# xinpw8/pokegym

Hardware: NVIDIA B200
Metric: env_steps_per_s (higher is better)
Workload: dtype u8

## Files before the change

pokegym_b200/csrc/gb_classes.inc:

```
#if defined(GB_CLS)
GB_CLS(0, 4, 0x2000u)
GB_CLS(1, 6, 0x1000u)
GB_CLS(2, 11, 0x0000u)
GB_CLS(3, 2, 0x4020u)
GB_CLS(4, 0, 0x0800u)
GB_CLS(5, 0, 0x0a00u)
GB_CLS(6, 3, 0x0000u)
GB_CLS(7, 0, 0x08a0u)
GB_CLS(8, 1, 0x0020u)
GB_CLS(9, 2, 0x4010u)
GB_CLS(10, 0, 0x0810u)
GB_CLS(11, 1, 0x0000u)
GB_CLS(12, 3, 0x0010u)
GB_CLS(13, 0, 0x0a80u)
GB_CLS(14, 0, 0x0820u)
GB_CLS(15, 9, 0x0000u)
GB_CLS(16, 10, 0x0160u)
GB_CLS(17, 1, 0x0200u)
GB_CLS(18, 8, 0x0160u)
GB_CLS(19, 7, 0x0000u)
GB_CLS(20, 3, 0x0020u)
GB_CLS(21, 4, 0x2220u)
GB_CLS(22, 8, 0x0560u)
GB_CLS(23, 12, 0x0000u)
GB_CLS(24, 2, 0x4000u)
GB_CLS(25, 14, 0x0000u)
GB_CLS(26, 5, 0x0000u)
GB_CLS(27, 15, 0x0000u)
GB_CLS(28, 13, 0x0000u)
GB_CLS(29, 16, 0x0000u)
GB_CLS(30, 0, 0x0a10u)
GB_CLS(31, 11, 0x0220u)
GB_CLS(32, 12, 0x0020u)
GB_CLS(33, 13, 0x0220u)
#endif
#define GB_CLS_COUNT 34
#define GB_CLS_DISPATCH(c, L, OTHER) \
if (GB_CLS_TEST((c) < 3u)) { \
    if (GB_CLS_TEST((c) == 0u)) { \
      L(0, 4, 0x2000u) \
    } else { \
        if (GB_CLS_TEST((c) == 1u)) { \
          L(1, 6, 0x1000u) \
        } else { \
              L(2, 11, 0x0000u) \
        } \
    } \
} else { \
    if (GB_CLS_TEST((c) < 6u)) { \
        if (GB_CLS_TEST((c) == 3u)) { \
          L(3, 2, 0x4020u) \
        } else { \
            if (GB_CLS_TEST((c) == 4u)) { \
              L(4, 0, 0x0800u) \
            } else { \
                  L(5, 0, 0x0a00u) \
            } \
        } \
    } else { \
        if (GB_CLS_TEST((c) < 8u)) { \
            if (GB_CLS_TEST((c) == 6u)) { \
              L(6, 3, 0x0000u) \
            } else { \
                  L(7, 0, 0x08a0u) \
            } \
        } else { \
            if (GB_CLS_TEST((c) < 11u)) { \
                if (GB_CLS_TEST((c) == 8u)) { \
                  L(8, 1, 0x0020u) \
                } else { \
                    if (GB_CLS_TEST((c) == 9u)) { \
                      L(9, 2, 0x4010u) \
                    } else { \
                          L(10, 0, 0x0810u) \
                    } \
                } \
            } else { \
                if (GB_CLS_TEST((c) < 14u)) { \
                    if (GB_CLS_TEST((c) == 11u)) { \
                      L(11, 1, 0x0000u) \
                    } else { \
                        if (GB_CLS_TEST((c) == 12u)) { \
                          L(12, 3, 0x0010u) \
                        } else { \
                              L(13, 0, 0x0a80u) \
                        } \
                    } \
                } else { \
                    if (GB_CLS_TEST((c) < 17u)) { \
                        if (GB_CLS_TEST((c) == 14u)) { \
                          L(14, 0, 0x0820u) \
                        } else { \
                            if (GB_CLS_TEST((c) == 15u)) { \
                              L(15, 9, 0x0000u) \
                            } else { \
                                  L(16, 10, 0x0160u) \
                            } \
                        } \
                    } else { \
                        if (GB_CLS_TEST((c) < 20u)) { \
                            if (GB_CLS_TEST((c) == 17u)) { \
                              L(17, 1, 0x0200u) \
                            } else { \
                                if (GB_CLS_TEST((c) == 18u)) { \
                                  L(18, 8, 0x0160u) \
                                } else { \
                                      L(19, 7, 0x0000u) \
                                } \
                            } \
                        } else { \
                            if (GB_CLS_TEST((c) < 22u)) { \
                                if (GB_CLS_TEST((c) == 20u)) { \
                                  L(20, 3, 0x0020u) \
                                } else { \
                                      L(21, 4, 0x2220u) \
                                } \
                            } else { \
                                if (GB_CLS_TEST((c) == 22u)) { \
                                  L(22, 8, 0x0560u) \
                                } else { \
                                    if (GB_CLS_TEST((c) == 23u)) { \
                                      L(23, 12, 0x0000u) \
                                    } else { \
                                        if (GB_CLS_TEST((c) == 24u)) { \
                                          L(24, 2, 0x4000u) \
                                        } else { \
                                            if (GB_CLS_TEST((c) == 25u)) { \
                                              L(25, 14, 0x0000u) \
                                            } else { \
                                                if (GB_CLS_TEST((c) == 26u)) { \
                                                  L(26, 5, 0x0000u) \
                                                } else { \
                                                    if (GB_CLS_TEST((c) == 27u)) { \
                                                      L(27, 15, 0x0000u) \
                                                    } else { \
                                                        if (GB_CLS_TEST((c) == 28u)) { \
                                                          L(28, 13, 0x0000u) \
                                                        } else { \
                                                            if (GB_CLS_TEST((c) == 29u)) { \
                                                              L(29, 16, 0x0000u) \
                                                            } else { \
                                                                if (GB_CLS_TEST((c) < 33u)) { \
                                                                    if (GB_CLS_TEST((c) == 30u)) { \
                                                                      L(30, 0, 0x0a10u) \
                                                                    } else { \
                                                                        if (GB_CLS_TEST((c) == 31u)) { \
                                                                          L(31, 11, 0x0220u) \
                                                                        } else { \
                                                                              L(32, 12, 0x0020u) \
                                                                        } \
                                                                    } \
                                                                } else { \
                                                                    if (GB_CLS_TEST((c) == 33u)) { \
                                                                      L(33, 13, 0x0220u) \
                                                                    } else { \
                                                                      OTHER \
                                                                    } \
                                                                } \
                                                            } \
                                                        } \
                                                    } \
                                                } \
                                            } \
                                        } \
                                    } \
                                } \
                            } \
                        } \
                    } \
                } \
            } \
        } \
    } \
} \
```

pokegym_b200/csrc/gb_cpu.cuh:

```cuda
#pragma once
#include "gb_device.cuh"
#include "gb_predecode.h"

#if !defined(GB_TRACE_SLOT)
#define GB_TRACE_SLOT(kind, phys, dx, dw)
#endif

__constant__ uint4 c_base_desc[512];

#define MODE_ATTN 0x8000u
#define MODE_POST 0x10000u
#define MODE_DEFER 0x20000u

struct RunCtx {
    const uint4 *rom_dec;
    uint32_t bank_mask;
};

__device__ __forceinline__ uint32_t hot_mode(const Machine &m) {
    const uint32_t attn = m.halted | m.iq | (m.iflag & m.ie & 0x1F), post = m.halted;
    return (attn ? MODE_ATTN : 0u) | (post ? MODE_POST : 0u) | (m.defer_active ? MODE_DEFER : 0u);
}
#define TIMA_ON 0x04000000u
__device__ __forceinline__ int hot_rem(Machine &m, bool fresh) {
    int rem = lcd_deadline(m);
    if (m.tmr & TIMA_ON) {
        int rt = (int)timer_divider(M_TAC(m)) - (int)m.timac;
        if (fresh) rt = rt < 1 ? 1 : rt;
        rem = rt < rem ? rt : rem;
    }
    return rem;
}
__device__ __forceinline__ void time_sync(Machine &m, int rem) {
    const uint32_t e = (uint32_t)(m.t_sync - rem);
    m.clock += e;
    m.divc += e;
    if (m.tmr & TIMA_ON) m.timac += e;
    m.t_sync = rem;
}

__global__ void k_predecode_rom(const uint8_t *rom, uint32_t rom_len, uint4 *out) {
    uint32_t o = blockIdx.x * blockDim.x + threadIdx.x;
    if (o >= rom_len) return;
    uint32_t in_bank = o & 0x3FFF;
    if (in_bank >= 0x3FFD) {
        out[o] = make_uint4(H_SLOW, 0, 0x32103210u, PD_NO_CLASS_W);
        return;
    }
    uint32_t ins = rom[o] | (rom[o + 1] << 8) | (rom[o + 2] << 16);
    out[o] = pd_finish(c_base_desc[(ins & 0xFF) == 0xCB ? (256u | ((ins >> 8) & 0xFF)) : (ins & 0xFF)], ins, o < 0x4000 ? o : 0x4000 + in_bank);
}

__device__ GB_NOINLINE uint4 cpu_decode_slow(Machine &m, uint32_t pc) {
    uint32_t ins = 0;
    if (pc - 0xFF80u < 0x7Du) {
        const uint32_t i = MEM_HI + (pc - 0xFE00), w0 = mem_rd_word(m, i >> 2), w1 = mem_rd_word(m, (i >> 2) + 1), sh = (i & 3) * 8;
        ins = sh ? ((w0 >> sh) | (w1 << (32 - sh))) : w0;
    } else {
        for (uint32_t i = 0; i < 3; i++) ins |= bus_read_full(m, (pc + i) & 0xFFFF) << (8 * i);
    }
    return pd_finish(c_base_desc[(ins & 0xFF) == 0xCB ? (256u | ((ins >> 8) & 0xFF)) : (ins & 0xFF)], ins, pc);
}

__device__ GB_NOINLINE uint32_t cpu_attention(Machine &m) {
    if (!m.iq) {
        const uint32_t pending = m.iflag & m.ie & 0x1F;
        if (pending) {
            const uint32_t bit = pending & (0u - pending);
            if (m.halted) m.pc = (m.pc + 1) & 0xFFFF;
            if (m.ime) {
                m.iflag ^= bit;
                bus_write_full(m, (m.sp - 1) & 0xFFFF, m.pc >> 8);
                bus_write_full(m, (m.sp - 2) & 0xFFFF, m.pc & 0xFF);
                m.sp = (m.sp - 2) & 0xFFFF;
                m.pc = 0x40 + 8 * (31 - __clz(bit));
                m.ime = 0;
            }
            m.iq = 1;
            m.halted = 0;
            return 0;
        }
    } else if (m.halted) {
        m.halted = 0;
        m.pc = (m.pc + 1) & 0xFFFF;
    }
    if (m.halted) return 4u << 8;
    m.iq = 0;
    return 1;
}

__device__ GB_NOINLINE uint32_t cpu_post_slow(Machine &m, uint32_t cycles) {
    if (m.halted) {
        const bool sleeps_on = (m.lcdc & 0x80) && !(m.iflag & m.ie & 0x1F);
        const int a = sleeps_on ? lcd_deadline(m) : (int)(m.target - m.clock), b = timer_cycles_to_interrupt(m), c = a < b ? a : b;
        cycles = c < 0 ? 0u : (uint32_t)c;
        if ((m.tmr & 0x04000000u) && b <= 0 && !(m.iflag & m.ie & 0x1F)) {
            const uint32_t n = 0xFFu - M_TIMA(m);
            m.timac -= n * timer_divider(M_TAC(m));
            m.tmr |= 0xFF00u;
        }
    }
    timer_tick_tima(m, cycles);
    return cycles;
}


struct CpuRegs {
    uint32_t bcde, hlaf, sp, pc;
};

#define FAST_WR_NONE 0xFFFFFFFFu
#define FAST_WR_DROP 0xFFFFFFFEu
#define FAST_WR_BANK 0xFFFFFFFDu
#define FAST_WR_P1 0xFFFFFFFCu
__device__ __forceinline__ uint32_t mem_offset(uint32_t i) { return ((i >> 2) << 7) | (i & 3); }
__device__ __forceinline__ uint32_t fast_store_target(uint32_t a) {
    if (a - 0xC000u < 0x3E00u) return mem_offset(MEM_WRAM + (a & 0x1FFF));
    if (a - 0xFF80u < 0x7Fu || a - 0xFE00u < 0x100u) return mem_offset(MEM_HI + (a - 0xFE00));
    if (a - 0x8000u < 0x2000u) return mem_offset(MEM_VRAM + (a - 0x8000));
    if (a - 0x2000u < 0x2000u) return FAST_WR_BANK;
    if (a - 0xFF10u < 0x30u) return FAST_WR_DROP;
    if (a == 0xFF00u) return FAST_WR_P1;
    return FAST_WR_NONE;
}
__device__ __forceinline__ bool fast_plain_offset(uint32_t a, uint32_t &off) {
    const bool wram = a - 0xC000u < 0x3E00u, vram = a - 0x8000u < 0x2000u;
    const bool hi = (a - 0xFE00u < 0x100u) | (a - 0xFF80u < 0x7Fu);
    const uint32_t i = wram ? MEM_WRAM + (a & 0x1FFF) : a + (vram ? MEM_VRAM - 0x8000u : MEM_HI - 0xFE00u);
    off = mem_offset(i);
    return wram | vram | hi;
}
__device__ __forceinline__ uint32_t fast_load_u8(const uint8_t *base, uint32_t off, bool ok, uint32_t otherwise) {
#if defined(GB_HOSTSIM)
    return ok ? base[off] : otherwise;
#else
    uint32_t r = otherwise;
    asm volatile("{\n\t.reg .pred p;\n\tsetp.ne.u32 p, %2, 0;\n\t@p ld.global.u8 %0, [%1];\n\t}" : "+r"(r) : "l"(base + off), "r"((uint32_t)ok) : "memory");
    return r;
#endif
}
__device__ __forceinline__ bool fast_stack_push(uint32_t sp) { return sp - 0xC002u < 0x3DFFu; }

template <bool FAST, bool SIMT, int CH = -1, uint32_t CF = 0>
__device__ __forceinline__ bool cpu_exec(Machine &m, const uint4 d, CpuRegs &r, uint32_t &rom_off, uint32_t &mode, uint32_t &cyc, uint8_t *memb,
                                         const uint8_t *rom, uint32_t bank_mask, bool declined = false) {
    uint32_t bcde = r.bcde, hlaf = r.hlaf, sp = r.sp;
#define FAST_DECLINE()         \
    do {                       \
        if (!SIMT) return false; \
        declined = true;       \
    } while (0)
    auto rd8 = [&](uint32_t a) -> uint32_t {
        if (FAST) {
            if (a - 0xC000u < 0x3E00u) return memb[mem_offset(MEM_WRAM + (a & 0x1FFF))];
            if (a < 0x8000u) return __ldg(rom + (a + (a >> 14) * rom_off));
            if (a - 0xFF80u < 0x7Fu || a - 0xFF00u < 4u) return memb[mem_offset(MEM_HI + (a - 0xFE00))];
            declined = true;
            return 0;
        }
        return bus_read_full(m, a);
    };
    const uint32_t w = d.w, wf = CH >= 0 ? CF : d.w, h = CH >= 0 ? (uint32_t)CH : (d.x & 0xFF);
    uint32_t v = gb_prmt(bcde, hlaf, w);
    if (wf & PDF_IMM) v = d.y & 0xFFFFu;
    uint32_t wa = 0, wt = 0;
    if (wf & (PDF_RD | PDF_WR)) {
        wa = (wf & PDF_AIMM) ? (d.y & 0xFFFFu) : (gb_prmt(bcde, hlaf, w >> 16) & 0xFFFFu);
        if (wf & PDF_ASP) wa = sp;
        if (FAST && SIMT) {
            uint32_t off;
            const bool plain = fast_plain_offset(wa, off);
            if (wf & PDF_WR) {
                wt = plain ? off : (wa - 0x2000u < 0x2000u) ? FAST_WR_BANK : (wa - 0xFF10u < 0x30u) ? FAST_WR_DROP : wa == 0xFF00u ? FAST_WR_P1 : FAST_WR_NONE;
                if (wt == FAST_WR_NONE) FAST_DECLINE();
                if ((mode & MODE_DEFER) && (wa - 0x8000u < 0x2000u || wa - 0xFE00u < 0x100u)) FAST_DECLINE();
            }
            if (wf & PDF_RD) {
                const bool in_rom = wa < 0x8000u, ok = plain | in_rom | (wa - 0xFF00u < 4u);
                v = fast_load_u8(in_rom ? rom : memb, in_rom ? wa + (wa >> 14) * rom_off : off, ok, v);
                if (!ok) declined = true;
                if (wf & PDF_RD16) {
                    const uint32_t wb = (wa + 1) & 0xFFFF;
                    uint32_t off2;
                    const bool plain2 = fast_plain_offset(wb, off2), in_rom2 = wb < 0x8000u, ok2 = plain2 | in_rom2 | (wb - 0xFF00u < 4u);
                    v |= fast_load_u8(in_rom2 ? rom : memb, in_rom2 ? wb + (wb >> 14) * rom_off : off2, ok2, 0) << 8;
                    if (!ok2) declined = true;
                }
            }
        } else {
            if (FAST && (wf & PDF_WR)) {
                wt = fast_store_target(wa);
                if (wt == FAST_WR_NONE) FAST_DECLINE();
                if ((mode & MODE_DEFER) && (wa - 0x8000u < 0x2000u || wa - 0xFE00u < 0x100u)) FAST_DECLINE();
            }
            if (wf & PDF_RD) {
                v = rd8(wa);
                if (wf & PDF_RD16) v |= rd8((wa + 1) & 0xFFFF) << 8;
                if (FAST && declined) return false;
            }
        }
    }
    const uint32_t imm16 = d.y & 0xFFFFu, op = gb_prmt(d.x, 0, 0x4441), ex = gb_prmt(d.x, 0, 0x4442), f = hlaf >> 24;
    uint32_t rv = v, next_pc = d.y >> 16, wv = v, wn = wf & PDF_WR;
    cyc = d.x >> 24;
#define PAIR_OPERAND() (gb_prmt(bcde, hlaf, w >> 16) & 0xFFFFu)
    const bool jump_taken = SIMT && (wf & PDF_JUMP) && ((f ^ ex) & op) == 0;
    if (SIMT) {
        next_pc = jump_taken ? imm16 : next_pc;
        cyc += jump_taken ? (ex & 0xF) : 0u;
    }
    if ((wf & PDF_MOV) || (SIMT && (wf & PDF_JUMP)) || (FAST && SIMT && declined)) {
    } else if (!SIMT && (wf & PDF_JUMP)) {
        if (((f ^ ex) & op) == 0) { next_pc = imm16; cyc += ex & 0xF; }
    } else if (!SIMT && (wf & PDF_INCDEC)) {
        const uint32_t b = v & 0xFF, sum = b + op, res = sum & 0xFF;
        const uint32_t nf = (f & FLAG_C) | ((((b ^ op ^ sum) & 0x10) << 1) ^ ex) | (res == 0 ? FLAG_Z : 0);
        rv = res | (nf << 8);
        wv = res;
    } else if (wf & (PDF_INCDEC | PDF_ARITH)) {
        const bool inc = SIMT && (wf & PDF_INCDEC) != 0;
        const uint32_t b = v & 0xFF;
        const uint32_t a = inc ? b : ((hlaf >> 16) & 0xFF), x = inc ? op : (b ^ ex);
        const uint32_t cin = inc ? 0u : ((((f >> 4) & op) ^ ex) & 1);
        const uint32_t sum = a + x + cin, res = sum & 0xFF;
        const uint32_t hn = (((a ^ x ^ sum) & 0x10) << 1) ^ (ex & 0x60);
        const uint32_t cb = inc ? (f & FLAG_C) : (((sum >> 4) ^ ex) & 0x10);
        rv = res | ((hn | cb | (res == 0 ? FLAG_Z : 0)) << 8);
        wv = res;
    } else if (h == H_HLI) {
        rv = ((PAIR_OPERAND() + gb_prmt(d.x, 0, 0x9991)) & 0xFFFFu) | (v << 16);
    } else switch (h) {
    case H_LOGIC: {
        const uint32_t a = (hlaf >> 16) & 0xFF, b = v & 0xFF;
        const uint32_t res = ((a & b) & ex) | ((a ^ b) & op);
        rv = res | (((op ? 0 : FLAG_H) | (res == 0 ? FLAG_Z : 0)) << 8);
        break;
    }
    case H_ADD_HL: {
        const uint32_t hl = hlaf & 0xFFFF, ar = PAIR_OPERAND(), t = hl + ar;
        const uint32_t nf = (f & FLAG_Z) | (((hl & 0xFFF) + (ar & 0xFFF)) > 0xFFF ? FLAG_H : 0) | (t > 0xFFFF ? FLAG_C : 0);
        rv = (t & 0xFFFF) | (nf << 24);
        break;
    }
    case H_CALL: {
        if (((f ^ ex) & op) == 0) {
            if (FAST && !fast_stack_push(sp)) FAST_DECLINE();
            wa = (sp - 1) & 0xFFFF;
            if (FAST) wt = mem_offset(MEM_WRAM + (wa & 0x1FFF));
            wv = gb_prmt(next_pc, 0, 0x4401);
            wn = 2;
            sp = (sp - 2) & 0xFFFF;
            next_pc = imm16;
            cyc += ex & 0xF;
        }
        break;
    }
    case H_RET: {
        if (wf & PDF_RETI) m.ime = 1;
        if (((f ^ ex) & op) == 0) {
            next_pc = v & 0xFFFF;
            sp = (sp + 2) & 0xFFFF;
            cyc += ex & 0xF;
        }
        break;
    }
    case H_PUSH:
        if (FAST && !fast_stack_push(sp)) FAST_DECLINE();
        wa = (sp - 1) & 0xFFFF;
        if (FAST) wt = mem_offset(MEM_WRAM + (wa & 0x1FFF));
        wv = gb_prmt(PAIR_OPERAND(), 0, 0x4401);
        wn = 2;
        sp = (sp - 2) & 0xFFFF;
        break;
    case H_POP:
        rv = v & (0xFF00u | op);
        sp = (sp + 2) & 0xFFFF;
        break;
    case H_ROT: {
        const uint32_t b = v & 0xFF, c = (f >> 4) & 1, right = ex & 1, b7 = b >> 7;
        uint32_t cout = right ? (b & 1) : b7;
        const uint32_t in = (((ex >> 1) & cout) | ((ex >> 2) & c) | ((ex >> 3) & b7)) & 1;
        uint32_t res = right ? ((b >> 1) | (in << 7)) : (((b << 1) | in) & 0xFF);
        if (ex & 0x10) { res = ((b >> 4) | (b << 4)) & 0xFF; cout = 0; }
        const uint32_t nf = ((res == 0 && !(op & 8)) ? FLAG_Z : 0) | (cout << 4);
        rv = res | (nf << 8);
        wv = res;
        break;
    }
    case H_CPL: rv = (~(hlaf >> 16) & 0xFF) | ((f | FLAG_N | FLAG_H) << 8); break;
    case H_IME: m.ime = op; break;
    case H_JPHL: next_pc = hlaf & 0xFFFF; break;
    case H_BIT: rv = ((f & FLAG_C) | FLAG_H | ((v & imm16 & 0xFF) ? 0 : FLAG_Z)) << 8; break;
    case H_RESSET:
        rv = (v & imm16 & 0xFF) | (imm16 >> 8);
        wv = rv;
        break;
    default: {
        if (FAST) {
            FAST_DECLINE();
            break;
        }
        const uint32_t a = (hlaf >> 16) & 0xFF, hl = hlaf & 0xFFFF;
        switch (op) {
        case 0x76: m.halted = 1; mode |= MODE_ATTN | MODE_POST; next_pc = r.pc; break;
        case 0x10: break;
        case 0xF3: m.ime = 0; break;
        case 0xFB: m.ime = 1; break;
        case 0x27: {
            uint32_t corr = ((f & FLAG_H) ? 0x06 : 0) | ((f & FLAG_C) ? 0x60 : 0), t = a;
            if (f & FLAG_N) {
                t -= corr;
            } else {
                if ((t & 0x0F) > 9) corr |= 0x06;
                if (t > 0x99) corr |= 0x60;
                t += corr;
            }
            t &= 0xFF;
            hlaf = (hlaf & 0xFFFF) | (t << 16) | (((f & FLAG_N) | (t == 0 ? FLAG_Z : 0) | ((corr & 0x60) ? FLAG_C : 0)) << 24);
            break;
        }
        case 0x2F: hlaf = (hlaf & 0xFFFF) | ((~a & 0xFF) << 16) | ((f | FLAG_N | FLAG_H) << 24); break;
        case 0x37: hlaf = (hlaf & 0x00FFFFFFu) | (((f & FLAG_Z) | FLAG_C) << 24); break;
        case 0x3F: hlaf = (hlaf & 0x00FFFFFFu) | (((f & FLAG_Z) | ((f & FLAG_C) ^ FLAG_C)) << 24); break;
        case 0x08: wa = imm16; wv = sp; wn = 3; break;
        case 0xE8:
        case 0xF8: {
            const uint32_t imm8 = imm16 & 0xFF;
            const uint32_t nf = (((sp & 0xF) + (imm8 & 0xF)) > 0xF ? FLAG_H : 0) | (((sp & 0xFF) + imm8) > 0xFF ? FLAG_C : 0);
            const uint32_t t = (sp + ((imm8 ^ 0x80) - 0x80)) & 0xFFFF;
            hlaf = (hlaf & 0x00FFFFFFu) | (nf << 24);
            if (op == 0xE8) sp = t;
            else hlaf = (hlaf & 0xFFFF0000u) | t;
            break;
        }
        case 0xE9: next_pc = hl; break;
        case 0xF9: sp = hl; break;
        case 0x31: sp = imm16; break;
        case 0x33: sp = (sp + 1) & 0xFFFF; break;
        case 0x3B: sp = (sp + 0xFFFF) & 0xFFFF; break;
        case 0x39: {
            const uint32_t t = hl + sp;
            const uint32_t nf = (f & FLAG_Z) | (((hl & 0xFFF) + (sp & 0xFFF)) > 0xFFF ? FLAG_H : 0) | (t > 0xFFFF ? FLAG_C : 0);
            hlaf = (hlaf & 0x00FF0000u) | (t & 0xFFFF) | (nf << 24);
            break;
        }
        case 0xE2: wa = 0xFF00u | (bcde & 0xFF); wv = a; wn = PDF_WR; break;
        case 0xF2: hlaf = (hlaf & 0xFF00FFFFu) | (bus_read_full(m, 0xFF00u | (bcde & 0xFF)) << 16); break;
        default: m.fault = 1; break;
        }
        break;
    }
    }
#undef PAIR_OPERAND
#if !defined(GB_HOSTSIM) && !defined(GB_OPT_NO_JOIN)
    if (FAST && SIMT) {
        uint32_t dj = declined;
        asm volatile("" : "+r"(dj));
        declined = dj != 0;
    }
#endif
    if (FAST && declined) return false;
#undef FAST_DECLINE
    r.bcde = gb_prmt(bcde, rv, d.z);
    r.hlaf = gb_prmt(hlaf, rv, d.z >> 16);
    r.sp = sp;
    r.pc = next_pc;
    if (wn) {
        if (FAST) {
            if (wt < FAST_WR_P1) {
                memb[wt] = (uint8_t)wv;
                if (wn == 2) memb[mem_offset(MEM_WRAM + ((wa - 1) & 0x1FFF))] = (uint8_t)(wv >> 8);
            } else if (wt == FAST_WR_P1) {
                memb[mem_offset(MEM_HI + 0x100)] = (uint8_t)joypad_pull(m, wv & 0xFF);
            } else if (wt == FAST_WR_BANK) {
                uint32_t bank = wv & 0x7F;
                bank = bank ? bank : 1;
                m.rombank = bank;
                rom_off = (bank_mask ? (bank & bank_mask) : (bank % m.rom_banks)) * 0x4000u - 0x4000u;
                m.rom_off = rom_off;
            }
        } else {
            const uint32_t count = (wn & 3) ? 2u : 1u, second = (wn == 2 ? wa - 1 : wa + 1) & 0xFFFF;
            for (uint32_t i = 0; i < count; i++) bus_write_full(m, i ? second : wa, (i ? wv >> 8 : wv) & 0xFF);
        }
    }
    return true;
}

__device__ __forceinline__ void gb_opaque(uint32_t &v) {
#if !defined(GB_HOSTSIM)
    asm volatile("" : "+r"(v));
#endif
}
__device__ __forceinline__ bool cpu_exec_by_class(Machine &m, const uint4 d, CpuRegs &r, uint32_t &rom_off, uint32_t &mode, uint32_t &cyc, uint8_t *memb,
                                                  const uint8_t *rom, uint32_t bank_mask) {
    uint32_t c = PD_CLASS(d.w);
#define GB_CLS_TEST(t) (gb_opaque(c), (t))
#define GB_CLS_RUN(id, H, F) return cpu_exec<true, false, H, F>(m, d, r, rom_off, mode, cyc, memb, rom, bank_mask);
    GB_CLS_DISPATCH(c, GB_CLS_RUN, return false;)
#undef GB_CLS_RUN
#undef GB_CLS_TEST
}

__device__ __forceinline__ bool cpu_exec_lockstep(Machine &m, const uint4 d, CpuRegs &r, uint32_t &rom_off, uint32_t mode, uint32_t &cyc, uint8_t *memb,
                                                  const uint8_t *rom, uint32_t bank_mask, bool declined) {
    const uint32_t bcde = r.bcde, hlaf = r.hlaf, sp = r.sp;
    const uint32_t w = d.w, h = d.x & 0xFF, op = gb_prmt(d.x, 0, 0x4441), ex = gb_prmt(d.x, 0, 0x4442), imm16 = d.y & 0xFFFFu, fall = d.y >> 16;
    const uint32_t f = hlaf >> 24, a8 = (hlaf >> 16) & 0xFF, hl = hlaf & 0xFFFF;
    declined |= h >= H_RARE;
    const bool cond = ((f ^ ex) & op) == 0;
    const bool is_call = h == H_CALL, is_ret = h == H_RET, is_push = h == H_PUSH, is_pop = h == H_POP;
    const bool jumps = cond && ((w & PDF_JUMP) || is_call), returns = cond && is_ret, pushes = (cond && is_call) || is_push;
    uint32_t v = gb_prmt(bcde, hlaf, w);
    v = (w & PDF_IMM) ? imm16 : v;
    const uint32_t pair = gb_prmt(bcde, hlaf, w >> 16) & 0xFFFFu;
    uint32_t wa = (w & PDF_AIMM) ? imm16 : pair;
    wa = (w & PDF_ASP) ? sp : wa;
    wa = pushes ? ((sp - 1) & 0xFFFF) : wa;
    uint32_t off;
    const bool plain = fast_plain_offset(wa, off);
    const bool rd = (w & PDF_RD) != 0, rd16 = (w & PDF_RD16) != 0, wr = (w & PDF_WR) != 0;
    const bool wr_special = wr && !plain;
    const uint32_t wt = (wa - 0x2000u < 0x2000u) ? FAST_WR_BANK : (wa - 0xFF10u < 0x30u) ? FAST_WR_DROP : wa == 0xFF00u ? FAST_WR_P1 : FAST_WR_NONE;
    declined |= wr_special && wt == FAST_WR_NONE;
    declined |= pushes && !fast_stack_push(sp);
    declined |= wr && (mode & MODE_DEFER) && (wa - 0x8000u < 0x2000u || wa - 0xFE00u < 0x100u);
    const bool in_rom = wa < 0x8000u, rd_ok = plain || in_rom || (wa - 0xFF00u < 4u), rd16_ok = sp - 0xC000u < 0x3DFFu;
    declined |= (rd && !rd_ok) || (rd16 && !rd16_ok);
    v = fast_load_u8(in_rom ? rom : memb, in_rom ? wa + (wa >> 14) * rom_off : off, rd && rd_ok, v);
    v |= fast_load_u8(memb, mem_offset(MEM_WRAM + ((sp + 1) & 0x1FFF)), rd16 && rd16_ok, 0) << 8;
    const uint32_t b = v & 0xFF, b7 = b >> 7;
    const bool inc = (w & PDF_INCDEC) != 0;
    const uint32_t ad_a = inc ? b : a8, ad_x = inc ? op : (b ^ ex), ad_c = inc ? 0u : ((((f >> 4) & op) ^ ex) & 1);
    const uint32_t sum = ad_a + ad_x + ad_c, ad_res = sum & 0xFF;
    const uint32_t ad_f = ((((ad_a ^ ad_x ^ sum) & 0x10) << 1) ^ (ex & 0x60)) | (inc ? (f & FLAG_C) : (((sum >> 4) ^ ex) & 0x10)) | (ad_res == 0 ? FLAG_Z : 0);
    const uint32_t lg_res = ((a8 & b) & ex) | ((a8 ^ b) & op);
    const uint32_t lg_f = (op ? 0 : FLAG_H) | (lg_res == 0 ? FLAG_Z : 0);
    const uint32_t right = ex & 1;
    uint32_t rt_c = right ? (b & 1) : b7;
    const uint32_t rt_in = (((ex >> 1) & rt_c) | ((ex >> 2) & (f >> 4)) | ((ex >> 3) & b7)) & 1;
    uint32_t rt_res = right ? ((b >> 1) | (rt_in << 7)) : (((b << 1) | rt_in) & 0xFF);
    rt_res = (ex & 0x10) ? (((b >> 4) | (b << 4)) & 0xFF) : rt_res;
    rt_c = (ex & 0x10) ? 0u : rt_c;
    const uint32_t rt_f = ((rt_res == 0 && !(op & 8)) ? FLAG_Z : 0) | (rt_c << 4);
    const uint32_t hli = ((pair + gb_prmt(d.x, 0, 0x9991)) & 0xFFFFu) | (v << 16);
    const uint32_t t16 = hl + pair;
    const uint32_t addhl = (t16 & 0xFFFF) | (((f & FLAG_Z) | (((hl & 0xFFF) + (pair & 0xFFF)) > 0xFFF ? FLAG_H : 0) | (t16 > 0xFFFF ? FLAG_C : 0)) << 24);
    uint32_t rv = v;
    rv = (w & (PDF_INCDEC | PDF_ARITH)) ? (ad_res | (ad_f << 8)) : rv;
    rv = h == H_LOGIC ? (lg_res | (lg_f << 8)) : rv;
    rv = h == H_ROT ? (rt_res | (rt_f << 8)) : rv;
    rv = h == H_BIT ? (((f & FLAG_C) | FLAG_H | ((b & imm16) ? 0 : FLAG_Z)) << 8) : rv;
    rv = h == H_RESSET ? ((b & imm16) | (imm16 >> 8)) : rv;
    rv = h == H_CPL ? ((~a8 & 0xFF) | ((f | FLAG_N | FLAG_H) << 8)) : rv;
    rv = h == H_HLI ? hli : rv;
    rv = h == H_ADD_HL ? addhl : rv;
    rv = is_pop ? (v & (0xFF00u | op)) : rv;
    uint32_t next_pc = jumps ? imm16 : fall;
    next_pc = returns ? (v & 0xFFFF) : next_pc;
    next_pc = h == H_JPHL ? hl : next_pc;
    cyc = (d.x >> 24) + ((jumps || returns) ? (ex & 0xF) : 0u);
    const uint32_t new_sp = (sp + ((is_pop || returns) ? 2u : 0u) - (pushes ? 2u : 0u)) & 0xFFFF;
    uint32_t wv = h == H_HLI ? v : rv;
    wv = pushes ? gb_prmt(is_push ? pair : fall, 0, 0x4401) : wv;
    if (declined) return false;
    r.bcde = gb_prmt(bcde, rv, d.z);
    r.hlaf = gb_prmt(hlaf, rv, d.z >> 16);
    r.sp = new_sp;
    r.pc = next_pc;
    if ((wr && plain) || pushes) memb[off] = (uint8_t)wv;
    if (pushes) memb[mem_offset(MEM_WRAM + ((sp - 2) & 0x1FFF))] = (uint8_t)(wv >> 8);
    if (wr_special) {
        if (wt == FAST_WR_P1) {
            memb[mem_offset(MEM_HI + 0x100)] = (uint8_t)joypad_pull(m, wv & 0xFF);
        } else if (wt == FAST_WR_BANK) {
            uint32_t bank = wv & 0x7F;
            bank = bank ? bank : 1;
            m.rombank = bank;
            rom_off = (bank_mask ? (bank & bank_mask) : (bank % m.rom_banks)) * 0x4000u - 0x4000u;
            m.rom_off = rom_off;
        }
    }
    if ((w & PDF_RETI) || h == H_IME) m.ime = h == H_IME ? op : 1u;
    return true;
}

__device__ GB_NOINLINE uint32_t cpu_tick_slow(Machine &m, const uint4 *__restrict__ rom_dec, uint32_t bank_mask, uint32_t &timer_ticked) {
    uint32_t cyc = 0;
    bool execute = true;
    if (m.halted | m.iq | (m.iflag & m.ie & 0x1F)) {
        const uint32_t r = cpu_attention(m);
        execute = r & 1;
        cyc = r >> 8;
    }
    if (execute) {
        const uint32_t pc = m.pc;
        uint4 d = make_uint4(H_SLOW, 0, 0, PD_NO_CLASS_W);
        if (pc < 0x8000u) d = __ldg(rom_dec + (pc + (pc >> 14) * m.rom_off));
        if ((d.x & 0xFF) == H_SLOW) d = cpu_decode_slow(m, pc);
        CpuRegs r = {m.bcde, m.hlaf, m.sp, pc};
        uint32_t rom_off = m.rom_off, mode = 0;
        cpu_exec<false, false>(m, d, r, rom_off, mode, cyc, m.memb, m.rom, bank_mask);
        m.bcde = r.bcde; m.hlaf = r.hlaf; m.sp = r.sp; m.pc = r.pc;
        m.n_instr++;
    }
    timer_ticked = m.halted;
    if (m.halted) cyc = cpu_post_slow(m, cyc);
    return cyc;
}

__device__ __forceinline__ uint4 cpu_decode_hram(const uint8_t *memb, uint32_t pc) {
    const uint32_t i = MEM_HI + (pc - 0xFE00), sh = (i & 3) * 8;
    const uint32_t w0 = ((const uint32_t *)memb)[(i >> 2) << 5], w1 = ((const uint32_t *)memb)[((i >> 2) + 1) << 5];
    const uint32_t ins = sh ? ((w0 >> sh) | (w1 << (32 - sh))) : w0;
    return pd_finish(c_base_desc[(ins & 0xFF) == 0xCB ? (256u | ((ins >> 8) & 0xFF)) : (ins & 0xFF)], ins, pc);
}

template <bool SIMT, bool CLASSES>
__device__ __forceinline__ bool cpu_fast_loop(Machine &m, const RunCtx &cx, CpuRegs &r, uint32_t &rom_off, uint32_t &mode, uint32_t &n_instr, int &rem,
                                              uint8_t *memb, const uint8_t *rom) {
    for (;;) {
        uint32_t cyc;
        uint4 d = make_uint4(H_SLOW, 0, 0x32103210u, PD_NO_CLASS_W);
        bool leave = false;
        const uint32_t pc = r.pc;
        if (!((pc | mode) & (0x8000u | MODE_POST))) {
            d = __ldg(cx.rom_dec + (pc + (pc >> 14) * rom_off));
        } else if (!(mode & (MODE_ATTN | MODE_POST)) && pc - 0xFF80u < 0x7Du) {
            d = cpu_decode_hram(memb, pc);
        } else {
            if (!SIMT) return false;
            leave = true;
        }
        if (SIMT) {
#if !defined(GB_OPT_LOCKSTEP)
            if (!cpu_exec<true, true>(m, d, r, rom_off, mode, cyc, memb, rom, cx.bank_mask, leave)) return false;
#else
            if (!cpu_exec_lockstep(m, d, r, rom_off, mode, cyc, memb, rom, cx.bank_mask, leave)) return false;
#endif
        } else if (CLASSES) {
            if (!cpu_exec_by_class(m, d, r, rom_off, mode, cyc, memb, rom, cx.bank_mask)) return false;
        } else {
            if (!cpu_exec<true, false>(m, d, r, rom_off, mode, cyc, memb, rom, cx.bank_mask, leave)) return false;
        }
        GB_TRACE_SLOT(0, pc < 0x8000u ? pc + (pc >> 14) * rom_off : (0xF00000u | pc), d.x, d.w);
        n_instr++;
        rem -= (int)cyc;
        if (rem <= 0) return true;
    }
}

template <bool SIMT>
__device__ __forceinline__ void cpu_run_to_event(Machine &m, const RunCtx &cx) {
    CpuRegs r = {m.bcde, m.hlaf, m.sp, m.pc};
    uint32_t rom_off = m.rom_off, n_instr = m.n_instr;
    uint8_t *memb = m.memb;
    const uint8_t *rom = m.rom;
    int rem = hot_rem(m, true);
    m.t_sync = rem;
    uint32_t mode = hot_mode(m), timer_pending = 0;
again:
    do {
        bool at_deadline;
        if (!SIMT && !(m.tmr & TIMA_ON)) at_deadline = cpu_fast_loop<SIMT, true>(m, cx, r, rom_off, mode, n_instr, rem, memb, rom);
        else at_deadline = cpu_fast_loop<SIMT, false>(m, cx, r, rom_off, mode, n_instr, rem, memb, rom);
        if (at_deadline) {
            timer_pending = 1;
            goto deadline;
        }
        {
            m.bcde = r.bcde; m.hlaf = r.hlaf; m.sp = r.sp; m.pc = r.pc; m.n_instr = n_instr;
            time_sync(m, rem);
            if (m.lazy && (int)(m.clock - m.target) >= 0) lcd_catch_up(m);
            GB_TRACE_SLOT(1, m.pc < 0x8000u ? m.pc + (m.pc >> 14) * m.rom_off : (0xF00000u | m.pc), 0, 0);
            uint32_t timer_ticked;
            const uint32_t cyc = cpu_tick_slow(m, cx.rom_dec, cx.bank_mask, timer_ticked);
            r.bcde = m.bcde; r.hlaf = m.hlaf; r.sp = m.sp; r.pc = m.pc; n_instr = m.n_instr; rom_off = m.rom_off;
            memb = m.memb; rom = m.rom;
            if (timer_ticked && (m.tmr & TIMA_ON)) m.timac -= cyc;
            timer_pending = !timer_ticked;
            rem = hot_rem(m, false);
            m.t_sync = rem;
            mode = hot_mode(m);
            rem -= (int)cyc;
        }
    } while (rem > 0);
deadline:
    m.bcde = r.bcde; m.hlaf = r.hlaf; m.sp = r.sp; m.pc = r.pc; m.n_instr = n_instr;
    time_sync(m, rem);
    if (timer_pending) timer_tick_tima(m, 0);
    if ((m.tmr & TIMA_ON) && !m.halted) {
        const bool lcd_due = (m.lcdc & 0x80) ? (int)(m.clock - m.target) >= 0 : m.clock >= FRAME_CYCLES;
        if (!lcd_due) {
            rem = hot_rem(m, true);
            m.t_sync = rem;
            mode = hot_mode(m);
            timer_pending = 0;
            if (rem > 0) goto again;
        }
    }
}
```

pokegym_b200/csrc/gb_predecode.h:

```cpp
#pragma once
#include <stdint.h>

enum {
    H_MOV = 0,
    H_HLI,
    H_ARITH,
    H_LOGIC,
    H_INCDEC,
    H_ADD_HL,
    H_JUMP,
    H_CALL,
    H_RET,
    H_PUSH,
    H_POP,
    H_ROT,
    H_BIT,
    H_RESSET,
    H_CPL,
    H_IME,
    H_JPHL,
    H_RARE,
    H_SLOW,
    H__COUNT
};

#define PDF_IMM 0x0010u
#define PDF_RD 0x0020u
#define PDF_RD16 0x0040u
#define PDF_AIMM 0x0080u
#define PDF_ASP 0x0100u
#define PDF_WR 0x0200u
#define PDF_RETI 0x0400u
#define PDF_MOV 0x0800u
#define PDF_JUMP 0x1000u
#define PDF_INCDEC 0x2000u
#define PDF_ARITH 0x4000u

#define PD_H(x) ((x) & 0xFFu)
#define PD_OP(x) (((x) >> 8) & 0xFFu)
#define PD_EX(x) (((x) >> 16) & 0xFFu)
#define PD_CYC(x) ((x) >> 24)

#if defined(__VECTOR_TYPES_H__)
typedef uint4 pd_desc_t;
#else
struct pd_desc_t { uint32_t x, y, z, w; };
#endif

enum { PDK_CONST = 0, PDK_IMM8, PDK_IMM16, PDK_JR, PDK_LDH };
#define PD_BASE_LEN(y) (((y) >> 16) & 3u)
#define PD_BASE_KIND(y) ((y) >> 24)

static inline uint32_t pd_reg_byte(uint32_t idx) { return ((idx & 4) ? 4u : 0u) + ((idx ^ 1u) & 3u); }

struct pd_builder {
    uint32_t h, cyc, ex, op, imm, len, kind, sel_lo, sel_hi, srcsel, flags, asel;
};
static inline void pd_b_init(pd_builder *b, uint32_t h, uint32_t len, uint32_t cyc) {
    b->h = h; b->cyc = cyc; b->ex = 0; b->op = 0; b->imm = 0; b->len = len; b->kind = PDK_CONST;
    b->sel_lo = 0x3210; b->sel_hi = 0x3210; b->srcsel = 0; b->flags = 0; b->asel = 0x5454;
}
static inline void pd_b_write(pd_builder *b, uint32_t k, uint32_t j) {
    uint32_t *sel = k < 4 ? &b->sel_lo : &b->sel_hi;
    uint32_t sh = (k & 3) * 4;
    *sel = (*sel & ~(0xFu << sh)) | ((4u + j) << sh);
}
static inline void pd_b_src_reg(pd_builder *b, uint32_t idx) { b->srcsel = pd_reg_byte(idx); }
static inline void pd_b_pair(pd_builder *b, uint32_t p) {
    static const uint32_t s[3] = {0x1010, 0x3232, 0x5454};
    b->asel = s[p];
}
static inline void pd_b_write_pair(pd_builder *b, uint32_t p) {
    pd_b_write(b, p * 2, 0);
    pd_b_write(b, p * 2 + 1, 1);
}
static inline uint32_t pd_class_id(uint32_t h, uint32_t flags) {
#if !defined(GB_NO_CLASS_LOOKUP)
#define GB_CLS(id, H, F) \
    if (h == (H) && flags == (F)) return id;
#include "gb_classes.inc"
#undef GB_CLS
#endif
    (void)h; (void)flags;
    return 0xFFu;
}
#define PD_CLASS(w) ((w) >> 24)
#define PD_NO_CLASS_W 0xFF000000u

static inline pd_desc_t pd_b_done(const pd_builder *b) {
    pd_desc_t d;
    d.x = b->h | (b->op << 8) | (b->ex << 16) | (b->cyc << 24);
    d.y = (b->imm & 0xFFFFu) | (b->len << 16) | (b->kind << 24);
    d.z = b->sel_lo | (b->sel_hi << 16);
    d.w = (b->srcsel & 0xFu) | (b->flags & 0xFFF0u) | (b->h == H_MOV ? PDF_MOV : 0u) | (b->h == H_JUMP ? PDF_JUMP : 0u) |
          (b->h == H_INCDEC ? PDF_INCDEC : 0u) | (b->h == H_ARITH ? PDF_ARITH : 0u) | ((b->asel & 0xFFu) << 16);
    d.w |= pd_class_id(b->h, d.w & 0xFFF0u) << 24;
    return d;
}

static inline void pd_b_cond(pd_builder *b, uint32_t cc, uint32_t taken_extra) {
    uint32_t mask = (cc & 2) ? 0x10u : 0x80u;
    b->op = mask;
    b->ex = taken_extra | ((cc & 1) ? mask : 0u);
}

static inline uint32_t pd_rot_ex(uint32_t y) {
    static const uint32_t t[8] = {0x02, 0x03, 0x04, 0x05, 0x00, 0x09, 0x10, 0x01};
    return t[y & 7];
}

static inline void pd_b_alu(pd_builder *b, uint32_t y) {
    if (y >= 4 && y <= 6) {
        b->h = H_LOGIC;
        b->ex = y == 5 ? 0u : 0xFFu;
        b->op = y == 4 ? 0u : 0xFFu;
    } else {
        b->h = H_ARITH;
        b->ex = (y == 2 || y == 3 || y == 7) ? 0xFFu : 0u;
        b->op = (y == 1 || y == 3) ? 1u : 0u;
    }
}

static inline void pd_build_base(pd_desc_t *t) {
    for (uint32_t opc = 0; opc < 256; opc++) {
        const uint32_t x = opc >> 6, y = (opc >> 3) & 7, z = opc & 7, p = y >> 1, q = y & 1;
        pd_builder b;
        pd_b_init(&b, H_RARE, 1, 4);
        b.op = opc;
        if (x == 1) {
            if (opc != 0x76) {
                pd_b_init(&b, H_MOV, 1, (y == 6 || z == 6) ? 8 : 4);
                if (z == 6) b.flags |= PDF_RD;
                else pd_b_src_reg(&b, z);
                if (y == 6) b.flags |= PDF_WR;
                else pd_b_write(&b, pd_reg_byte(y), 0);
            }
        } else if (x == 2) {
            pd_b_init(&b, H_ARITH, 1, z == 6 ? 8 : 4);
            pd_b_alu(&b, y);
            if (z == 6) b.flags |= PDF_RD;
            else pd_b_src_reg(&b, z);
            if (y != 7) pd_b_write(&b, 6, 0);
            pd_b_write(&b, 7, 1);
        } else if (x == 0) {
            switch (z) {
            case 0:
                if (y == 0) {
                    pd_b_init(&b, H_MOV, 1, 4);
                } else if (y == 1) {
                    b.len = 3; b.cyc = 20; b.kind = PDK_IMM16;
                } else if (y == 2) {
                    b.len = 2;
                } else {
                    pd_b_init(&b, H_JUMP, 2, y == 3 ? 12 : 8);
                    b.kind = PDK_JR;
                    if (y >= 4) pd_b_cond(&b, y & 3, 4);
                }
                break;
            case 1:
                if (q == 0) {
                    if (p == 3) { b.len = 3; b.cyc = 12; b.kind = PDK_IMM16; }
                    else {
                        pd_b_init(&b, H_MOV, 3, 12);
                        b.kind = PDK_IMM16; b.flags |= PDF_IMM;
                        pd_b_write_pair(&b, p);
                    }
                } else {
                    if (p == 3) { b.cyc = 8; }
                    else {
                        pd_b_init(&b, H_ADD_HL, 1, 8);
                        pd_b_pair(&b, p);
                        pd_b_write(&b, 4, 0); pd_b_write(&b, 5, 1); pd_b_write(&b, 7, 3);
                    }
                }
                break;
            case 2: {
                pd_b_init(&b, p < 2 ? H_MOV : H_HLI, 1, 8);
                pd_b_pair(&b, p < 2 ? p : 2);
                if (p >= 2) b.op = p == 2 ? 1u : 0xFFu;
                if (q == 0) {
                    b.srcsel = 6; b.flags |= PDF_WR;
                    if (p >= 2) { pd_b_write(&b, 4, 0); pd_b_write(&b, 5, 1); }
                } else {
                    b.flags |= PDF_RD;
                    if (p >= 2) { pd_b_write(&b, 4, 0); pd_b_write(&b, 5, 1); pd_b_write(&b, 6, 2); }
                    else pd_b_write(&b, 6, 0);
                }
                break;
            }
            case 3:
                if (p == 3) { b.cyc = 8; }
                else {
                    pd_b_init(&b, H_HLI, 1, 8);
                    pd_b_pair(&b, p);
                    b.op = q ? 0xFFu : 1u;
                    pd_b_write_pair(&b, p);
                }
                break;
            case 4:
            case 5:
                pd_b_init(&b, H_INCDEC, 1, y == 6 ? 12 : 4);
                b.op = (z & 1) ? 0xFFu : 1u;
                b.ex = (z & 1) ? 0x60u : 0u;
                if (y == 6) b.flags |= PDF_RD | PDF_WR;
                else { pd_b_src_reg(&b, y); pd_b_write(&b, pd_reg_byte(y), 0); }
                pd_b_write(&b, 7, 1);
                break;
            case 6:
                pd_b_init(&b, H_MOV, 2, y == 6 ? 12 : 8);
                b.kind = PDK_IMM8; b.flags |= PDF_IMM;
                if (y == 6) b.flags |= PDF_WR;
                else pd_b_write(&b, pd_reg_byte(y), 0);
                break;
            default:
                if (y < 4) {
                    pd_b_init(&b, H_ROT, 1, 4);
                    b.op = y | 8u; b.ex = pd_rot_ex(y); b.srcsel = 6;
                    pd_b_write(&b, 6, 0); pd_b_write(&b, 7, 1);
                }
                else if (y == 5) {
                    pd_b_init(&b, H_CPL, 1, 4);
                    pd_b_write(&b, 6, 0); pd_b_write(&b, 7, 1);
                }
                break;
            }
        } else {
            switch (z) {
            case 0:
                if (y < 4) {
                    pd_b_init(&b, H_RET, 1, 8);
                    b.flags |= PDF_RD | PDF_RD16 | PDF_ASP;
                    pd_b_cond(&b, y, 12);
                } else if (y == 4 || y == 6) {
                    pd_b_init(&b, H_MOV, 2, 12);
                    b.kind = PDK_LDH; b.flags |= PDF_AIMM;
                    if (y == 4) { b.srcsel = 6; b.flags |= PDF_WR; }
                    else { b.flags |= PDF_RD; pd_b_write(&b, 6, 0); }
                } else {
                    b.len = 2; b.cyc = y == 5 ? 16 : 12; b.kind = PDK_IMM8;
                }
                break;
            case 1:
                if (q == 0) {
                    pd_b_init(&b, H_POP, 1, 12);
                    b.flags |= PDF_RD | PDF_RD16 | PDF_ASP;
                    b.op = p == 3 ? 0xF0u : 0xFFu;
                    if (p == 3) { pd_b_write(&b, 6, 1); pd_b_write(&b, 7, 0); }
                    else pd_b_write_pair(&b, p);
                } else if (p < 2) {
                    pd_b_init(&b, H_RET, 1, 16);
                    b.flags |= PDF_RD | PDF_RD16 | PDF_ASP | (p == 1 ? PDF_RETI : 0);
                } else if (p == 3) {
                    b.cyc = 8;
                } else {
                    pd_b_init(&b, H_JPHL, 1, 4);
                }
                break;
            case 2:
                if (y < 4) {
                    pd_b_init(&b, H_JUMP, 3, 12);
                    b.kind = PDK_IMM16;
                    pd_b_cond(&b, y, 4);
                } else if (y == 4 || y == 6) {
                    b.cyc = 8;
                } else {
                    pd_b_init(&b, H_MOV, 3, 16);
                    b.kind = PDK_IMM16; b.flags |= PDF_AIMM;
                    if (y == 5) { b.srcsel = 6; b.flags |= PDF_WR; }
                    else { b.flags |= PDF_RD; pd_b_write(&b, 6, 0); }
                }
                break;
            case 3:
                if (y == 0) { pd_b_init(&b, H_JUMP, 3, 16); b.kind = PDK_IMM16; }
                else if (y == 6 || y == 7) { pd_b_init(&b, H_IME, 1, 4); b.op = y & 1; }
                break;
            case 4:
                if (y < 4) {
                    pd_b_init(&b, H_CALL, 3, 12);
                    b.kind = PDK_IMM16;
                    pd_b_cond(&b, y, 12);
                }
                break;
            case 5:
                if (q == 0) {
                    pd_b_init(&b, H_PUSH, 1, 16);
                    if (p == 3) b.asel = 0x6767;
                    else pd_b_pair(&b, p);
                } else if (p == 0) {
                    pd_b_init(&b, H_CALL, 3, 24);
                    b.kind = PDK_IMM16;
                }
                break;
            case 6:
                pd_b_init(&b, H_ARITH, 2, 8);
                pd_b_alu(&b, y);
                b.kind = PDK_IMM8; b.flags |= PDF_IMM;
                if (y != 7) pd_b_write(&b, 6, 0);
                pd_b_write(&b, 7, 1);
                break;
            default:
                pd_b_init(&b, H_CALL, 1, 16);
                b.imm = y * 8;
                break;
            }
        }
        t[opc] = pd_b_done(&b);
    }
    for (uint32_t opc = 0; opc < 256; opc++) {
        const uint32_t x = opc >> 6, y = (opc >> 3) & 7, z = opc & 7;
        pd_builder b;
        pd_b_init(&b, x == 0 ? H_ROT : x == 1 ? H_BIT : H_RESSET, 2, z == 6 ? 16 : 8);
        if (z == 6) b.flags |= PDF_RD | (x == 1 ? 0 : PDF_WR);
        else pd_b_src_reg(&b, z);
        if (x == 0) {
            b.op = y; b.ex = pd_rot_ex(y);
            pd_b_write(&b, 7, 1);
        } else if (x == 1) {
            b.imm = 1u << y;
            pd_b_write(&b, 7, 1);
        } else {
            b.imm = x == 2 ? (0xFFu & ~(1u << y)) : (0xFFu | ((1u << y) << 8));
        }
        if (x != 1 && z != 6) pd_b_write(&b, pd_reg_byte(z), 0);
        t[256 + opc] = pd_b_done(&b);
    }
}

#if defined(__CUDACC__)
__host__ __device__
#endif
static inline pd_desc_t pd_finish(pd_desc_t b, uint32_t ins, uint32_t pc) {
    const uint32_t imm16 = (ins >> 8) & 0xFFFFu, imm8 = imm16 & 0xFFu, len = PD_BASE_LEN(b.y);
    uint32_t imm = b.y & 0xFFFFu;
    switch (PD_BASE_KIND(b.y)) {
    case PDK_IMM8: imm = imm8; break;
    case PDK_IMM16: imm = imm16; break;
    case PDK_JR: imm = (pc + 2 + ((imm8 ^ 0x80u) - 0x80u)) & 0xFFFFu; break;
    case PDK_LDH: imm = 0xFF00u | imm8; break;
    default: break;
    }
    b.y = imm | (((pc + len) & 0xFFFFu) << 16);
    return b;
}
```

Baseline: 191,500.

## Add dedicated class-dispatch interpreter loop with per-case continuation and skip register writeback

```diff
diff --git a/pokegym_b200/csrc/gb_classes.inc b/pokegym_b200/csrc/gb_classes.inc
--- a/pokegym_b200/csrc/gb_classes.inc
+++ b/pokegym_b200/csrc/gb_classes.inc
@@ -36,122 +36,122 @@
 #endif
 #define GB_CLS_COUNT 34
 #define GB_CLS_DISPATCH(c, L, OTHER) \
-if (GB_CLS_TEST((c) < 3u)) { \
-    if (GB_CLS_TEST((c) == 0u)) { \
+if (GB_CLS_BELOW(c, 3u)) { \
+    if (GB_CLS_BELOW(c, 1u)) { \
       L(0, 4, 0x2000u) \
     } else { \
-        if (GB_CLS_TEST((c) == 1u)) { \
+        if (GB_CLS_BELOW(c, 2u)) { \
           L(1, 6, 0x1000u) \
         } else { \
               L(2, 11, 0x0000u) \
         } \
     } \
 } else { \
-    if (GB_CLS_TEST((c) < 6u)) { \
-        if (GB_CLS_TEST((c) == 3u)) { \
+    if (GB_CLS_BELOW(c, 6u)) { \
+        if (GB_CLS_BELOW(c, 4u)) { \
           L(3, 2, 0x4020u) \
         } else { \
-            if (GB_CLS_TEST((c) == 4u)) { \
+            if (GB_CLS_BELOW(c, 5u)) { \
               L(4, 0, 0x0800u) \
             } else { \
                   L(5, 0, 0x0a00u) \
             } \
         } \
     } else { \
-        if (GB_CLS_TEST((c) < 8u)) { \
-            if (GB_CLS_TEST((c) == 6u)) { \
+        if (GB_CLS_BELOW(c, 8u)) { \
+            if (GB_CLS_BELOW(c, 7u)) { \
               L(6, 3, 0x0000u) \
             } else { \
                   L(7, 0, 0x08a0u) \
             } \
         } else { \
-            if (GB_CLS_TEST((c) < 11u)) { \
-                if (GB_CLS_TEST((c) == 8u)) { \
+            if (GB_CLS_BELOW(c, 11u)) { \
+                if (GB_CLS_BELOW(c, 9u)) { \
                   L(8, 1, 0x0020u) \
                 } else { \
-                    if (GB_CLS_TEST((c) == 9u)) { \
+                    if (GB_CLS_BELOW(c, 10u)) { \
                       L(9, 2, 0x4010u) \
                     } else { \
                           L(10, 0, 0x0810u) \
                     } \
                 } \
             } else { \
-                if (GB_CLS_TEST((c) < 14u)) { \
-                    if (GB_CLS_TEST((c) == 11u)) { \
+                if (GB_CLS_BELOW(c, 14u)) { \
+                    if (GB_CLS_BELOW(c, 12u)) { \
                       L(11, 1, 0x0000u) \
                     } else { \
-                        if (GB_CLS_TEST((c) == 12u)) { \
+                        if (GB_CLS_BELOW(c, 13u)) { \
                           L(12, 3, 0x0010u) \
                         } else { \
                               L(13, 0, 0x0a80u) \
                         } \
                     } \
                 } else { \
-                    if (GB_CLS_TEST((c) < 17u)) { \
-                        if (GB_CLS_TEST((c) == 14u)) { \
+                    if (GB_CLS_BELOW(c, 17u)) { \
+                        if (GB_CLS_BELOW(c, 15u)) { \
                           L(14, 0, 0x0820u) \
                         } else { \
-                            if (GB_CLS_TEST((c) == 15u)) { \
+                            if (GB_CLS_BELOW(c, 16u)) { \
                               L(15, 9, 0x0000u) \
                             } else { \
                                   L(16, 10, 0x0160u) \
                             } \
                         } \
                     } else { \
-                        if (GB_CLS_TEST((c) < 20u)) { \
-                            if (GB_CLS_TEST((c) == 17u)) { \
+                        if (GB_CLS_BELOW(c, 20u)) { \
+                            if (GB_CLS_BELOW(c, 18u)) { \
                               L(17, 1, 0x0200u) \
                             } else { \
-                                if (GB_CLS_TEST((c) == 18u)) { \
+                                if (GB_CLS_BELOW(c, 19u)) { \
                                   L(18, 8, 0x0160u) \
                                 } else { \
                                       L(19, 7, 0x0000u) \
                                 } \
                             } \
                         } else { \
-                            if (GB_CLS_TEST((c) < 22u)) { \
-                                if (GB_CLS_TEST((c) == 20u)) { \
+                            if (GB_CLS_BELOW(c, 22u)) { \
+                                if (GB_CLS_BELOW(c, 21u)) { \
                                   L(20, 3, 0x0020u) \
                                 } else { \
                                       L(21, 4, 0x2220u) \
                                 } \
                             } else { \
-                                if (GB_CLS_TEST((c) == 22u)) { \
+                                if (GB_CLS_BELOW(c, 23u)) { \
                                   L(22, 8, 0x0560u) \
                                 } else { \
-                                    if (GB_CLS_TEST((c) == 23u)) { \
+                                    if (GB_CLS_BELOW(c, 24u)) { \
                                       L(23, 12, 0x0000u) \
                                     } else { \
-                                        if (GB_CLS_TEST((c) == 24u)) { \
+                                        if (GB_CLS_BELOW(c, 25u)) { \
                                           L(24, 2, 0x4000u) \
                                         } else { \
-                                            if (GB_CLS_TEST((c) == 25u)) { \
+                                            if (GB_CLS_BELOW(c, 26u)) { \
                                               L(25, 14, 0x0000u) \
                                             } else { \
-                                                if (GB_CLS_TEST((c) == 26u)) { \
+                                                if (GB_CLS_BELOW(c, 27u)) { \
                                                   L(26, 5, 0x0000u) \
                                                 } else { \
-                                                    if (GB_CLS_TEST((c) == 27u)) { \
+                                                    if (GB_CLS_BELOW(c, 28u)) { \
                                                       L(27, 15, 0x0000u) \
                                                     } else { \
-                                                        if (GB_CLS_TEST((c) == 28u)) { \
+                                                        if (GB_CLS_BELOW(c, 29u)) { \
                                                           L(28, 13, 0x0000u) \
                                                         } else { \
-                                                            if (GB_CLS_TEST((c) == 29u)) { \
+                                                            if (GB_CLS_BELOW(c, 30u)) { \
                                                               L(29, 16, 0x0000u) \
                                                             } else { \
-                                                                if (GB_CLS_TEST((c) < 33u)) { \
-                                                                    if (GB_CLS_TEST((c) == 30u)) { \
+                                                                if (GB_CLS_BELOW(c, 33u)) { \
+                                                                    if (GB_CLS_BELOW(c, 31u)) { \
                                                                       L(30, 0, 0x0a10u) \
                                                                     } else { \
-                                                                        if (GB_CLS_TEST((c) == 31u)) { \
+                                                                        if (GB_CLS_BELOW(c, 32u)) { \
                                                                           L(31, 11, 0x0220u) \
                                                                         } else { \
                                                                               L(32, 12, 0x0020u) \
                                                                         } \
                                                                     } \
                                                                 } else { \
-                                                                    if (GB_CLS_TEST((c) == 33u)) { \
+                                                                    if (GB_CLS_BELOW(c, 34u)) { \
                                                                       L(33, 13, 0x0220u) \
                                                                     } else { \
                                                                       OTHER \
diff --git a/pokegym_b200/csrc/gb_cpu.cuh b/pokegym_b200/csrc/gb_cpu.cuh
--- a/pokegym_b200/csrc/gb_cpu.cuh
+++ b/pokegym_b200/csrc/gb_cpu.cuh
@@ -361,8 +361,10 @@
 #endif
     if (FAST && declined) return false;
 #undef FAST_DECLINE
-    r.bcde = gb_prmt(bcde, rv, d.z);
-    r.hlaf = gb_prmt(hlaf, rv, d.z >> 16);
+    if (!(CH == H_JUMP || CH == H_CALL || CH == H_RET || CH == H_PUSH || CH == H_IME || CH == H_JPHL)) {
+        r.bcde = gb_prmt(bcde, rv, d.z);
+        r.hlaf = gb_prmt(hlaf, rv, d.z >> 16);
+    }
     r.sp = sp;
     r.pc = next_pc;
     if (wn) {
@@ -391,15 +393,6 @@
 #if !defined(GB_HOSTSIM)
     asm volatile("" : "+r"(v));
 #endif
-}
-__device__ __forceinline__ bool cpu_exec_by_class(Machine &m, const uint4 d, CpuRegs &r, uint32_t &rom_off, uint32_t &mode, uint32_t &cyc, uint8_t *memb,
-                                                  const uint8_t *rom, uint32_t bank_mask) {
-    uint32_t c = PD_CLASS(d.w);
-#define GB_CLS_TEST(t) (gb_opaque(c), (t))
-#define GB_CLS_RUN(id, H, F) return cpu_exec<true, false, H, F>(m, d, r, rom_off, mode, cyc, memb, rom, bank_mask);
-    GB_CLS_DISPATCH(c, GB_CLS_RUN, return false;)
-#undef GB_CLS_RUN
-#undef GB_CLS_TEST
 }
 
 __device__ __forceinline__ bool cpu_exec_lockstep(Machine &m, const uint4 d, CpuRegs &r, uint32_t &rom_off, uint32_t mode, uint32_t &cyc, uint8_t *memb,
@@ -516,7 +509,7 @@
     return pd_finish(c_base_desc[(ins & 0xFF) == 0xCB ? (256u | ((ins >> 8) & 0xFF)) : (ins & 0xFF)], ins, pc);
 }
 
-template <bool SIMT, bool CLASSES>
+template <bool SIMT>
 __device__ __forceinline__ bool cpu_fast_loop(Machine &m, const RunCtx &cx, CpuRegs &r, uint32_t &rom_off, uint32_t &mode, uint32_t &n_instr, int &rem,
                                               uint8_t *memb, const uint8_t *rom) {
     for (;;) {
@@ -538,8 +531,6 @@
 #else
             if (!cpu_exec_lockstep(m, d, r, rom_off, mode, cyc, memb, rom, cx.bank_mask, leave)) return false;
 #endif
-        } else if (CLASSES) {
-            if (!cpu_exec_by_class(m, d, r, rom_off, mode, cyc, memb, rom, cx.bank_mask)) return false;
         } else {
             if (!cpu_exec<true, false>(m, d, r, rom_off, mode, cyc, memb, rom, cx.bank_mask, leave)) return false;
         }
@@ -548,6 +539,40 @@
         rem -= (int)cyc;
         if (rem <= 0) return true;
     }
+}
+
+__device__ __forceinline__ bool cpu_class_loop(Machine &m, const RunCtx &cx, CpuRegs &r, uint32_t &rom_off, uint32_t &mode, uint32_t &n_instr, int &rem,
+                                               uint8_t *memb, const uint8_t *rom) {
+    __shared__ const uint4 *s_rom_dec;
+    s_rom_dec = cx.rom_dec;
+    const uint4 *const rom_dec = *(const uint4 *const volatile *)&s_rom_dec;
+    const uint32_t bank_mask = cx.bank_mask;
+    int t = -rem;
+    for (;;) {
+        const uint32_t pc = r.pc;
+        uint4 d;
+        if ((pc | mode) & (0x8000u | MODE_POST)) {
+            if ((mode & (MODE_ATTN | MODE_POST)) || pc - 0xFF80u >= 0x7Du) break;
+            d = cpu_decode_hram(memb, pc);
+        } else {
+            d = __ldg(rom_dec + (pc + (pc >> 14) * rom_off));
+        }
+        uint32_t cw = d.w, cyc;
+#define GB_CLS_BELOW(w, n) (gb_opaque(w), PD_CLASS_BELOW(w, n))
+#define GB_CLS_RUN(id, H, F)                                                                                   \
+    if (!cpu_exec<true, false, H, F>(m, d, r, rom_off, mode, cyc, memb, rom, bank_mask)) break;               \
+    GB_TRACE_SLOT(0, pc < 0x8000u ? pc + (pc >> 14) * rom_off : (0xF00000u | pc), d.x, d.w);                  \
+    n_instr++;                                                                                                 \
+    t += (int)cyc;                                                                                             \
+    if (t < 0) continue;                                                                                       \
+    rem = -t;                                                                                                  \
+    return true;
+        GB_CLS_DISPATCH(cw, GB_CLS_RUN, break;)
+#undef GB_CLS_RUN
+#undef GB_CLS_BELOW
+    }
+    rem = -t;
+    return false;
 }
 
 template <bool SIMT>
@@ -562,8 +587,8 @@
 again:
     do {
         bool at_deadline;
-        if (!SIMT && !(m.tmr & TIMA_ON)) at_deadline = cpu_fast_loop<SIMT, true>(m, cx, r, rom_off, mode, n_instr, rem, memb, rom);
-        else at_deadline = cpu_fast_loop<SIMT, false>(m, cx, r, rom_off, mode, n_instr, rem, memb, rom);
+        if (!SIMT && !(m.tmr & TIMA_ON)) at_deadline = cpu_class_loop(m, cx, r, rom_off, mode, n_instr, rem, memb, rom);
+        else at_deadline = cpu_fast_loop<SIMT>(m, cx, r, rom_off, mode, n_instr, rem, memb, rom);
         if (at_deadline) {
             timer_pending = 1;
             goto deadline;
diff --git a/pokegym_b200/csrc/gb_predecode.h b/pokegym_b200/csrc/gb_predecode.h
--- a/pokegym_b200/csrc/gb_predecode.h
+++ b/pokegym_b200/csrc/gb_predecode.h
@@ -85,6 +85,7 @@
     return 0xFFu;
 }
 #define PD_CLASS(w) ((w) >> 24)
+#define PD_CLASS_BELOW(w, m) ((w) < ((m) << 24))
 #define PD_NO_CLASS_W 0xFF000000u
 
 static inline pd_desc_t pd_b_done(const pd_builder *b) {
```

Result: faster. 202,800 (median of 6 runs) (+5.8%).
